# Siyou-Li/u2Tokenizer

Measured on NVIDIA H100. Metric: ct_volumes_per_sec, higher is better.
Workload: dtype bf16

## Files before the change

include/u2b200.h:

```cpp
#ifndef U2B200_H_
#define U2B200_H_

#include <stdint.h>

#if defined(__GNUC__)
#define U2_API __attribute__((visibility("default")))
#else
#define U2_API
#endif

#ifdef __cplusplus
extern "C" {
#endif

#define U2_OK 0
#define U2_ERR_ARG (-1)
#define U2_ERR_CUDA (-2)
#define U2_ERR_UNSUPPORTED (-3)

#define U2_DT_BF16 0
#define U2_DT_F32 1

#define U2_ACT_NONE 0
#define U2_ACT_GELU 1
// ... 97 lines not shown
} u2_rope_desc;
U2_API int u2_rope_bf16(void* x, const u2_rope_desc* desc, void* stream);

U2_API int u2_decode_attention_bf16(const void* q, const void* k_cache, const void* v_cache, void* out,
                                    int32_t B, int32_t Hq, int32_t Hkv, int32_t dh, int32_t Tmax, int32_t T,
                                    const int32_t* T_dev, int64_t ldq, int64_t ldo, float scale, int32_t T_per_seq,
                                    const int32_t* kv_src, int64_t ld_kv_src, void* stream);
U2_API int u2_decode_attention_window_bf16(const void* q, const void* k_cache, const void* v_cache, void* out,
                                           int32_t B, int32_t Hq, int32_t Hkv, int32_t dh, int32_t Tmax, int32_t T,
                                           const int32_t* T_dev, int64_t ldq, int64_t ldo, float scale,
                                           int32_t T_per_seq, const int32_t* kv_src, int64_t ld_kv_src,
                                           int32_t window, void* stream);

typedef struct u2_gemv_desc {
  int32_t B, N, K;
  int64_t ldx, ldw, ldy, ldr;
  int32_t y_dtype;
  const void* residual;
  const float* norm_gamma;
  float norm_eps;
  int32_t silu_pair;
} u2_gemv_desc;
U2_API int u2_gemv_bf16(const void* x, const void* w, void* y, const u2_gemv_desc* desc, void* stream);
U2_API int u2_argmax_f32(const float* logits, int64_t* out, uint64_t* scratch, int32_t B, int32_t V, int64_t ld,
                         void* stream);

#define U2_DLIN_STREAMK128 0
#define U2_DLIN_TILES64 1
typedef struct u2_dlinear_desc {
  int32_t B, N, K;
  int64_t ldx, ldw, ldy, ldr, ldxg;
  int32_t y_dtype;
  float* ws;
  int32_t* counters;
  const float* ssq_in;
  float eps;
  const void* residual;
  int32_t silu_pair;
  const float* gamma_next;
  void* xg;
  float* ssq_out;
  float* ssq_zero;
  int32_t pdl;
  void* dbg;
  int64_t ws_elems;
  const int32_t* dep_flags;
  int32_t dep_shift;
  int32_t* out_flags;
  int32_t sched;
} u2_dlinear_desc;
U2_API int u2_dlinear_bf16(const void* x, const void* w, void* y, const u2_dlinear_desc* desc, void* stream);
U2_API int64_t u2_dlinear_ws_elems(int32_t N, int32_t K);
typedef struct u2_dlinear_next {
  int32_t pre_stages;
  int32_t lookahead_units;
  int32_t n;
  const void* w[2];
  int32_t N[2], K[2];
  int64_t ldw[2];
  int32_t units[2];
} u2_dlinear_next;
U2_API int u2_dlinear_multi_bf16(const void* const* x, const void* const* w, void* const* y,
                                 const u2_dlinear_desc* descs, int32_t n_ops, uint32_t* gridbar,
                                 const int32_t* step_dev, int32_t pdl, const u2_dlinear_next* next, void* stream);
U2_API int u2_decode_embed_bf16(const int64_t* ids, const void* table, const float* gamma, void* x, void* xg,
                                float* ssq, float* ssq_zero, int32_t* step_counter, int32_t B, int32_t E,
                                int64_t vocab, void* stream);

typedef struct u2_fused_decode_desc {
  int32_t B, Hq, Hkv, dh, Tmax, pos;
  const int32_t* pos_dev;
  int64_t ldq, ldo;
  const float* q_norm_w;
  const float* k_norm_w;
  float eps;
  const float* inv_freq;
  float scale;
  int32_t kv_splits;
  int32_t pdl;
  int32_t pos_per_seq;
  const int32_t* kv_src;
  int64_t ld_kv_src;
  int32_t window;
} u2_fused_decode_desc;
U2_API int u2_decode_attention_fused_bf16(const void* qkv, void* k_cache, void* v_cache, void* out,
                                          const u2_fused_decode_desc* desc, void* stream);

U2_API int u2_topk_rows_f32(const float* scores, int64_t* out_idx, int32_t rows, int32_t T, int32_t K, int64_t ld,
                            int64_t idx_offset_per_row, void* stream);

typedef struct u2_fa_desc {
  int32_t B, H, Sq, Sk, dh;
  float scale;
  int64_t q_sb, q_ss, q_sh;
  int64_t k_sb, k_ss, k_sh;
  int64_t v_sb, v_ss, v_sh;
  int64_t out_sb, out_ss;
  float* lse;
} u2_fa_desc;
U2_API int u2_flash_attention_d64_bf16(const void* q, const void* k, const void* v, void* out, const u2_fa_desc* desc,
                                       void* stream);

U2_API int u2_sample_f32(const float* logits, int64_t* out, int32_t B, int32_t V, int64_t ld, float temperature,
                         int32_t top_k, float top_p, uint64_t seed, const int32_t* step_dev, int32_t step,
                         void* stream);

typedef struct u2_sample_params {
  float temperature;
  int32_t top_k;
  float top_p;
  int32_t reserved;
  uint64_t seed;
} u2_sample_params;
U2_API int u2_sample_dev_f32(const float* logits, int64_t* out, int32_t B, int32_t V, int64_t ld,
                             const u2_sample_params* params_dev, const int32_t* step_dev, int32_t step, void* stream);

#define U2_LP_MAX_EOS 8
#define U2_LP_MAX_BAD_WORDS 256
#define U2_LP_MAX_BAD_TOKENS 2048
typedef struct u2_logits_proc_params {
  float penalty;
  float inv_penalty;
  int32_t ngram;
  int32_t min_new;
  int32_t n_eos;
  int32_t n_bad;
  int32_t eos[U2_LP_MAX_EOS];
  int32_t bad_off[U2_LP_MAX_BAD_WORDS + 1];
  int32_t bad_tok[U2_LP_MAX_BAD_TOKENS];
} u2_logits_proc_params;
U2_API int u2_logits_process_f32(float* logits, int32_t B, int32_t V, int64_t ld, const int64_t* ids, int32_t* hist,
                                 int64_t ld_hist, int32_t hist_cap, const u2_logits_proc_params* params_dev,
                                 const int32_t* step_dev, int32_t step, void* stream);

#define U2_BEAM_MAX_BEAMS 16
#define U2_BEAM_MAX_EOS 8
#define U2_BEAM_MAX_KEEP 144
typedef struct u2_beam_params {
  double length_penalty;
  int32_t num_beams;
  int32_t beams_to_keep;
  int32_t early_stopping;
  int32_t max_new_tokens;
  int32_t n_eos;
  int32_t reserved;
  int32_t eos[U2_BEAM_MAX_EOS];
} u2_beam_params;
typedef struct u2_beam_step_desc {
  const u2_beam_params* params;
  int32_t prompts, V;
  const float* cand_val;
  const int32_t* cand_tok;
  float* running;
  float* fin_score;
  int32_t* fin_info;
  int32_t* flags;
  int64_t* ids;
  int32_t* rec;
  int64_t ld_rec;
  int32_t rec_rows;
  int32_t* kv_src;
  int64_t ld_kv_src;
  const int32_t* pos_dev;
  int32_t* hist;
  int64_t ld_hist;
  int32_t hist_cap;
// ... 50 lines not shown
```

u2tokenizer_b200/_lib.py:

```python
from __future__ import annotations

import ctypes as C
from pathlib import Path

_LIB_PATH = Path(__file__).resolve().parent / "libu2b200.so"
_lib = None


class GemmDesc(C.Structure):
    _fields_ = [
        ("M", C.c_int32), ("N", C.c_int32), ("K", C.c_int32),
        ("zi", C.c_int32), ("zo", C.c_int32), ("b_zi_div", C.c_int32),
        ("lda", C.c_int64), ("a_stride_zi", C.c_int64), ("a_stride_zo", C.c_int64),
        ("ldb", C.c_int64), ("b_stride_zi", C.c_int64), ("b_stride_zo", C.c_int64),
        ("ldc", C.c_int64), ("c_stride_zi", C.c_int64), ("c_stride_zo", C.c_int64),
        ("c_dtype", C.c_int32), ("alpha", C.c_float),
        ("bias", C.c_void_p),
        ("act", C.c_int32),
        ("residual", C.c_void_p),
        ("ldr", C.c_int64),
        ("res_row_mod", C.c_int32),
        ("row_div", C.c_int32), ("row_stride", C.c_int32), ("row_off", C.c_int32),
        ("block_n", C.c_int32),
        ("a_mn", C.c_int32), ("b_mn", C.c_int32),
        ("epi_op", C.c_int32),
        ("rowvec", C.c_void_p),
        ("rv_stride_zi", C.c_int64), ("rv_stride_zo", C.c_int64),
        ("mul", C.c_void_p),
    ]


class SoftmaxDesc(C.Structure):
    _fields_ = [
        ("in_s0", C.c_int64), ("in_s1", C.c_int64), ("in_s2", C.c_int64),
        ("out_s0", C.c_int64), ("out_s1", C.c_int64), ("out_s2", C.c_int64),
        ("n0", C.c_int32), ("H", C.c_int32), ("S", C.c_int32), ("n", C.c_int32),
        ("scale", C.c_float),
        ("rel_bias", C.c_void_p),
        ("rel_max", C.c_int32),
        ("causal", C.c_int32), ("causal_off", C.c_int32),
        ("zero_pad_to", C.c_int32),
        ("window", C.c_int32),
    ]


class RopeDesc(C.Structure):
    _fields_ = [
        ("rows", C.c_int64), ("ld", C.c_int64),
        ("dh", C.c_int32), ("n_q_heads", C.c_int32), ("n_k_heads", C.c_int32), ("n_v_heads", C.c_int32),
        ("q_norm_w", C.c_void_p), ("k_norm_w", C.c_void_p),
        ("eps", C.c_float),
        ("inv_freq", C.c_void_p),
        ("pos0", C.c_int32), ("pos_div", C.c_int32), ("pos_mod", C.c_int32),
        ("pos0_dev", C.c_void_p),
        ("k_cache", C.c_void_p), ("v_cache", C.c_void_p),
        ("Tmax", C.c_int32), ("rows_per_batch", C.c_int32),
        ("pos0_per_batch", C.c_int32),
    ]


class GemvDesc(C.Structure):
    _fields_ = [
        ("B", C.c_int32), ("N", C.c_int32), ("K", C.c_int32),
        ("ldx", C.c_int64), ("ldw", C.c_int64), ("ldy", C.c_int64), ("ldr", C.c_int64),
        ("y_dtype", C.c_int32),
        ("residual", C.c_void_p),
        ("norm_gamma", C.c_void_p),
        ("norm_eps", C.c_float),
        ("silu_pair", C.c_int32),
    ]


class DlinearDesc(C.Structure):
    _fields_ = [
        ("B", C.c_int32), ("N", C.c_int32), ("K", C.c_int32),
        ("ldx", C.c_int64), ("ldw", C.c_int64), ("ldy", C.c_int64), ("ldr", C.c_int64), ("ldxg", C.c_int64),
        ("y_dtype", C.c_int32),
        ("ws", C.c_void_p), ("counters", C.c_void_p),
        ("ssq_in", C.c_void_p),
        ("eps", C.c_float),
        ("residual", C.c_void_p),
        ("silu_pair", C.c_int32),
        ("gamma_next", C.c_void_p),
        ("xg", C.c_void_p),
        ("ssq_out", C.c_void_p),
        ("ssq_zero", C.c_void_p),
        ("pdl", C.c_int32),
        ("dbg", C.c_void_p),
        ("ws_elems", C.c_int64),
        ("dep_flags", C.c_void_p), ("dep_shift", C.c_int32), ("out_flags", C.c_void_p),
        ("sched", C.c_int32),
    ]


class FusedDecodeDesc(C.Structure):
    _fields_ = [
        ("B", C.c_int32), ("Hq", C.c_int32), ("Hkv", C.c_int32), ("dh", C.c_int32), ("Tmax", C.c_int32),
        ("pos", C.c_int32),
        ("pos_dev", C.c_void_p),
        ("ldq", C.c_int64), ("ldo", C.c_int64),
        ("q_norm_w", C.c_void_p), ("k_norm_w", C.c_void_p),
        ("eps", C.c_float),
        ("inv_freq", C.c_void_p),
        ("scale", C.c_float),
        ("kv_splits", C.c_int32), ("pdl", C.c_int32),
        ("pos_per_seq", C.c_int32),
        ("kv_src", C.c_void_p), ("ld_kv_src", C.c_int64),
        ("window", C.c_int32),
    ]


class DlinearNext(C.Structure):
    _fields_ = [
        ("pre_stages", C.c_int32), ("lookahead_units", C.c_int32), ("n", C.c_int32),
        ("w", C.c_void_p * 2),
        ("N", C.c_int32 * 2), ("K", C.c_int32 * 2),
        ("ldw", C.c_int64 * 2),
        ("units", C.c_int32 * 2),
    ]


class FaDesc(C.Structure):
    _fields_ = [
        ("B", C.c_int32), ("H", C.c_int32), ("Sq", C.c_int32), ("Sk", C.c_int32), ("dh", C.c_int32),
        ("scale", C.c_float),
        ("q_sb", C.c_int64), ("q_ss", C.c_int64), ("q_sh", C.c_int64),
        ("k_sb", C.c_int64), ("k_ss", C.c_int64), ("k_sh", C.c_int64),
        ("v_sb", C.c_int64), ("v_ss", C.c_int64), ("v_sh", C.c_int64),
        ("out_sb", C.c_int64), ("out_ss", C.c_int64),
        ("lse", C.c_void_p),
    ]


class LogprobDesc(C.Structure):
    _fields_ = [
        ("R", C.c_int32), ("V", C.c_int32), ("E", C.c_int32),
        ("ldh", C.c_int64), ("ldw", C.c_int64),
        ("labels", C.c_void_p), ("ws", C.c_void_p), ("ws_bytes", C.c_int64),
        ("lse", C.c_void_p), ("logit_sum", C.c_void_p), ("nll_acc", C.c_void_p),
    ]


class PreprocessInfo(C.Structure):
    _fields_ = [
        ("a_min", C.c_double), ("a_max", C.c_double),
        ("lo", C.c_int32 * 3), ("hi", C.c_int32 * 3), ("out", C.c_int32 * 3),
        ("sigma", C.c_float * 3), ("tail", C.c_int32 * 3), ("status", C.c_int32),
    ]


class PreprocessDesc(C.Structure):
    _fields_ = [
        ("D", C.c_int32), ("H", C.c_int32), ("W", C.c_int32), ("target", C.c_int32), ("pad_depth", C.c_int32),
        ("lower_pct", C.c_double), ("upper_pct", C.c_double),
        ("ws", C.c_void_p), ("ws_bytes", C.c_int64),
    ]


class SoftmaxBwdDesc(C.Structure):
    _fields_ = [
        ("p_s0", C.c_int64), ("p_s1", C.c_int64), ("p_s2", C.c_int64),
        ("dp_s0", C.c_int64), ("dp_s1", C.c_int64), ("dp_s2", C.c_int64),
        ("ds_s0", C.c_int64), ("ds_s1", C.c_int64), ("ds_s2", C.c_int64),
        ("n0", C.c_int32), ("H", C.c_int32), ("S", C.c_int32), ("n", C.c_int32),
        ("zero_pad_to", C.c_int32),
    ]


class AdamWDesc(C.Structure):
    _fields_ = [
        ("lr", C.c_float), ("beta1", C.c_float), ("beta2", C.c_float), ("eps", C.c_float), ("weight_decay", C.c_float),
        ("step", C.c_int32),
        ("grad_scale", C.c_void_p),
        ("seed", C.c_uint64), ("index_offset", C.c_int64),
    ]


class LoraDesc(C.Structure):
    _fields_ = [
        ("M", C.c_int32), ("K", C.c_int32), ("r", C.c_int32), ("n_adapters", C.c_int32),
        ("ldx", C.c_int64), ("ldu", C.c_int64),
        ("scale", C.c_float), ("p", C.c_float),
        ("seed", C.c_uint64),
        ("stream", C.c_int32 * 3),
        ("accumulate", C.c_int32),
    ]


LP_MAX_EOS, LP_MAX_BAD_WORDS, LP_MAX_BAD_TOKENS = 8, 256, 2048


# ... 154 lines not shown
```

u2tokenizer_b200/csrc/attn_small.cu:

```cuda
#include <cooperative_groups.h>
#include <cuda_bf16.h>
#include <math.h>

#include <type_traits>

#include "host_util.h"
#include "u2b200.h"

namespace u2 {

__device__ __forceinline__ float wsum(float v) {
#pragma unroll
  for (int o = 16; o > 0; o >>= 1) v += __shfl_xor_sync(0xffffffffu, v, o);
  return v;
}
__device__ __forceinline__ float wmax(float v) {
#pragma unroll
  for (int o = 16; o > 0; o >>= 1) v = fmaxf(v, __shfl_xor_sync(0xffffffffu, v, o));
  return v;
}

__global__ void __launch_bounds__(128)
temporal_attention_kernel(const __nv_bfloat16* __restrict__ qkv, __nv_bfloat16* __restrict__ out, int C, int N,
                          int H, int dh, long long ld_qkv, long long ld_out, float scale,
// ... 701 lines not shown
#pragma unroll
      for (int i = 0; i < kEpl; ++i) acc[g][i] *= corr;
      m[g] = mx;
    }
#pragma unroll
    for (int jj = 0; jj < 32; ++jj) {
      float vf[kEpl];
      if (t0 + jj == pos) {
#pragma unroll
        for (int i = 0; i < kEpl; ++i) vf[i] = __bfloat162float(s_vnew[le * kEpl + i]);
      } else if constexpr (kEpl == 4) {
        const float2 x = __bfloat1622float2(*reinterpret_cast<const __nv_bfloat162*>(&vw[jj][0]));
        const float2 y = __bfloat1622float2(*reinterpret_cast<const __nv_bfloat162*>(&vw[jj][1]));
        vf[0] = x.x; vf[1] = x.y; vf[2] = y.x; vf[3] = y.y;
      } else if constexpr (kEpl == 2) {
        const float2 x = __bfloat1622float2(*reinterpret_cast<const __nv_bfloat162*>(&vw[jj][0]));
        vf[0] = x.x; vf[1] = x.y;
      } else {
        vf[0] = __uint_as_float(vw[jj][0] << 16);
      }
#pragma unroll
      for (int g = 0; g < kG; ++g) {
        const float pj = __shfl_sync(0xffffffffu, p[g], jj);
#pragma unroll
        for (int i = 0; i < kEpl; ++i) acc[g][i] += pj * vf[i];
      }
    }
    t0 += S * kW * 32;
    if (t0 < T) request(t0);
  }
#pragma unroll
  for (int g = 0; g < kG; ++g) {
    if (lane == 0) {
      s_m[warp][g] = m[g];
      s_l[warp][g] = l[g];
    }
    if (kLanes == 32 || lane < kLanes) {
#pragma unroll
      for (int i = 0; i < kEpl; ++i) s_acc[warp][g][lane * kEpl + i] = acc[g][i];
    }
  }
  __syncthreads();
  for (int idx = threadIdx.x; idx < kG * kDh; idx += blockDim.x) {
    const int g = idx / kDh, e = idx - g * kDh;
    float gm = -INFINITY;
#pragma unroll
    for (int w = 0; w < kW; ++w) gm = fmaxf(gm, s_m[w][g]);
    float gl = 0.f, o = 0.f;
#pragma unroll
    for (int w = 0; w < kW; ++w) {
      if (s_m[w][g] != -INFINITY) {
        const float f = __expf(s_m[w][g] - gm);
        gl += s_l[w][g] * f;
        o += s_acc[w][g][e] * f;
      }
    }
    c_o[g][e] = o;
    if (e == 0) {
      c_m[g] = gm;
      c_l[g] = gl;
    }
  }
  cluster.sync();
  if (rank == 0) {
    for (int idx = threadIdx.x; idx < kG * kDh; idx += blockDim.x) {
      const int g = idx / kDh, e = idx - g * kDh;
      float gm = -INFINITY;
      for (int r = 0; r < S; ++r) gm = fmaxf(gm, *cluster.map_shared_rank(&c_m[g], r));
      float gl = 0.f, o = 0.f;
      for (int r = 0; r < S; ++r) {
        const float mr = *cluster.map_shared_rank(&c_m[g], r);
        if (mr != -INFINITY) {
          const float f = __expf(mr - gm);
          gl += *cluster.map_shared_rank(&c_l[g], r) * f;
          o += *cluster.map_shared_rank(&c_o[g][e], r) * f;
        }
      }
      a.out[(long long)b * a.ldo + (long long)(hk * kG + g) * kDh + e] = __float2bfloat16(o / gl);
    }
  }
  cluster.sync();
}

template <int kDh, int kG, bool kInd, bool kWin>
static int launch_fused_decode_split(const FusedArgsT<kInd, kWin>& a, dim3 grid, bool pdl, cudaStream_t st) {
  cudaLaunchConfig_t cfg = {};
  cfg.gridDim = grid;
  cfg.blockDim = dim3(256);
  cfg.dynamicSmemBytes = 0;
  cfg.stream = st;
  cudaLaunchAttribute attr[2];
  attr[0].id = cudaLaunchAttributeClusterDimension;
  attr[0].val.clusterDim.x = 1;
  attr[0].val.clusterDim.y = 1;
  attr[0].val.clusterDim.z = grid.z;
  attr[1].id = cudaLaunchAttributeProgrammaticStreamSerialization;
  attr[1].val.programmaticStreamSerializationAllowed = 1;
  cfg.attrs = attr;
  cfg.numAttrs = pdl ? 2 : 1;
  cudaError_t e = cudaLaunchKernelEx(&cfg, fused_decode_attention_split_kernel<kDh, kG, kInd, kWin>, a);
  if (e != cudaSuccess) return set_error(U2_ERR_CUDA, "decode_attention_fused (split-KV) launch: %s", cudaGetErrorString(e));
  return U2_OK;
}

template <int kDh, bool kInd, bool kWin = false>
static int launch_fused_decode(const FusedArgsT<kInd, kWin>& a, int G, dim3 grid, bool pdl, cudaStream_t st) {
  if (grid.z > 1) {
    switch (G) {
      case 1: return launch_fused_decode_split<kDh, 1, kInd, kWin>(a, grid, pdl, st);
      case 2: return launch_fused_decode_split<kDh, 2, kInd, kWin>(a, grid, pdl, st);
      case 4: return launch_fused_decode_split<kDh, 4, kInd, kWin>(a, grid, pdl, st);
      case 8: return launch_fused_decode_split<kDh, 8, kInd, kWin>(a, grid, pdl, st);
      default: return set_error(U2_ERR_UNSUPPORTED, "decode_attention_fused: Hq/Hkv = %d (supported 1, 2, 4, 8)", G);
    }
  }
  switch (G) {
    case 1: fused_decode_attention_kernel<kDh, 1, kInd, kWin><<<grid, FaCfg<kDh, 1>::kWarps * 32, 0, st>>>(a); break;
    case 2: fused_decode_attention_kernel<kDh, 2, kInd, kWin><<<grid, FaCfg<kDh, 2>::kWarps * 32, 0, st>>>(a); break;
    case 4: fused_decode_attention_kernel<kDh, 4, kInd, kWin><<<grid, FaCfg<kDh, 4>::kWarps * 32, 0, st>>>(a); break;
    case 8: fused_decode_attention_kernel<kDh, 8, kInd, kWin><<<grid, FaCfg<kDh, 8>::kWarps * 32, 0, st>>>(a); break;
    default: return set_error(U2_ERR_UNSUPPORTED, "decode_attention_fused: Hq/Hkv = %d (supported 1, 2, 4, 8)", G);
  }
  return U2_OK;
}

template <int kDh>
static int launch_fused_decode(const FusedDecodeWinArgs& a, int G, dim3 grid, bool pdl, cudaStream_t st) {
  if (a.window > 0) {
    if (a.kv_src) return launch_fused_decode<kDh, true, true>(a, G, grid, pdl, st);
    return launch_fused_decode<kDh, false, true>(a, G, grid, pdl, st);
  }
  if (a.kv_src) return launch_fused_decode<kDh, true>(static_cast<const FusedDecodeIndArgs&>(a), G, grid, pdl, st);
  return launch_fused_decode<kDh, false>(static_cast<const FusedDecodeArgs&>(a), G, grid, pdl, st);
}

}

extern "C" U2_API int u2_decode_attention_fused_bf16(const void* qkv, void* k_cache, void* v_cache, void* out,
                                                     const u2_fused_decode_desc* d, void* stream) {
  using namespace u2;
  if (!qkv || !k_cache || !v_cache || !out || !d || !d->inv_freq) return set_error(U2_ERR_ARG, "decode_attention_fused: null pointer");
  if (d->Hkv <= 0 || d->Hq % d->Hkv || d->Hq / d->Hkv > kFaMaxG)
    return set_error(U2_ERR_UNSUPPORTED, "decode_attention_fused: Hq/Hkv must be an integer <= %d", kFaMaxG);
  if (!d->pos_dev && (d->pos < 0 || d->pos >= d->Tmax)) return set_error(U2_ERR_ARG, "decode_attention_fused: position outside the cache");
  if (d->pos_per_seq && !d->pos_dev) return set_error(U2_ERR_ARG, "decode_attention_fused: pos_per_seq needs pos_dev");
  if (d->window < 0) return set_error(U2_ERR_ARG, "decode_attention_fused: window %d < 0", d->window);
  FusedDecodeWinArgs a;
  a.qkv = CBF(qkv); a.ldq = d->ldq;
  a.kc = BF(k_cache); a.vc = BF(v_cache);
  a.out = BF(out); a.ldo = d->ldo;
  a.Hq = d->Hq; a.Hkv = d->Hkv; a.Tmax = d->Tmax;
  a.pos_dev = d->pos_dev; a.pos_per_seq = d->pos_per_seq != 0; a.pos_host = d->pos;
  a.q_norm_w = d->q_norm_w; a.k_norm_w = d->k_norm_w; a.eps = d->eps;
  a.inv_freq = d->inv_freq; a.scale = d->scale;
  a.kv_src = d->kv_src; a.ld_src = d->ld_kv_src;
  a.window = d->window;
  if (a.kv_src && a.ld_src < d->Tmax) return set_error(U2_ERR_ARG, "decode_attention_fused: kv_src row stride < Tmax");
  const int splits = d->kv_splits > 1 ? d->kv_splits : 1;
  if (splits != 1 && splits != 2 && splits != 4 && splits != 8)
    return set_error(U2_ERR_ARG, "decode_attention_fused: kv_splits must be 0/1, 2, 4 or 8 (portable cluster sizes)");
  dim3 grid((unsigned)d->Hkv, (unsigned)d->B, (unsigned)splits);
  const int G = d->Hq / d->Hkv;
  int rc;
  switch (d->dh) {
    case 32: rc = launch_fused_decode<32>(a, G, grid, d->pdl != 0, ST(stream)); break;
    case 64: rc = launch_fused_decode<64>(a, G, grid, d->pdl != 0, ST(stream)); break;
    case 96: rc = launch_fused_decode<96>(a, G, grid, d->pdl != 0, ST(stream)); break;
    case 128: rc = launch_fused_decode<128>(a, G, grid, d->pdl != 0, ST(stream)); break;
    default: return set_error(U2_ERR_UNSUPPORTED, "decode_attention_fused: head_dim %d (supported 32/64/96/128)", d->dh);
  }
  if (rc) return rc;
  U2_CHECK_LAUNCH("decode_attention_fused");
  return U2_OK;
}
```

u2tokenizer_b200/engine.py:

```python
from __future__ import annotations

import math
from dataclasses import asdict, dataclass, replace
from typing import Dict, List, Optional, Tuple

import torch

from . import _lib, ops
from .geometry import Geometry

BF16, F32 = torch.bfloat16, torch.float32
REL_MAX = 512


def _pad8(n: int) -> int:
    return (n + 7) // 8 * 8


@dataclass(frozen=True)
class LogitsProcessors:
    repetition_penalty: float = 1.0
    no_repeat_ngram_size: int = 0
    min_new_tokens: int = 0
    eos_token_ids: Tuple[int, ...] = ()
# ... 540 lines not shown

    def token_logps(self, hidden: torch.Tensor, labels: torch.Tensor, *, want_lse=False, want_logit_sum=False,
                    nll_acc: Optional[torch.Tensor] = None):
        shp = labels.shape
        h2 = hidden.reshape(-1, hidden.shape[-1])
        if not h2.is_contiguous():
            h2 = h2.contiguous()
        logp, lse, lsum = ops.lmhead_logprob(h2, self.lm_head, labels.reshape(-1).contiguous(), want_lse=want_lse,
                                             want_logit_sum=want_logit_sum, nll_acc=nll_acc)
        rs = lambda t: None if t is None else t.view(shp)
        return rs(logp), rs(lse), rs(lsum)

    def _decode_buffers(self, B: int):
        g = self.g
        key = ("dec", B)
        if getattr(self, "_dec_key", None) != key:
            if getattr(self, "_gen_state", None) is not None:
                self._gen_state["graph"] = None
            hq, hkv, dh, I, E = g.num_attention_heads, g.num_key_value_heads, g.head_dim, g.intermediate_size, g.hidden_size
            d = self.dev
            self._dec = dict(
                x=torch.empty(B, E, device=d, dtype=BF16), qkv=torch.empty(B, (hq + 2 * hkv) * dh, device=d, dtype=BF16),
                ctx=torch.empty(B, hq * dh, device=d, dtype=BF16), act=torch.empty(B, I, device=d, dtype=BF16),
                logits=torch.empty(B, g.vocab_size, device=d, dtype=F32), ids=torch.zeros(B, 1, device=d, dtype=torch.int64),
                xg=torch.empty(B, E, device=d, dtype=BF16), xg2=torch.empty(B, E, device=d, dtype=BF16),
                ssq_a=torch.zeros(16, device=d, dtype=F32),
                ssq_b=torch.zeros(16, device=d, dtype=F32))
            max_n = max(g.vocab_size, 2 * I, (hq + 2 * hkv) * dh, E)
            shapes = [((hq + 2 * hkv) * dh, E), (E, hq * dh), (2 * I, E), (E, I), (g.vocab_size, E)]
            wse = max(ops.dlinear_ws_elems(n, k) for n, k in shapes)
            self._dec["ws"] = ops.dlinear_new_ws(wse, device=d, lead=(2,))
            self._dec["counters"] = torch.zeros(2, (max_n + 63) // 64 + 8, device=d, dtype=torch.int32)
            self._dec["flags"] = torch.zeros(g.num_hidden_layers, 4, 256, device=d, dtype=torch.int32)
            self._dec["gridbar"] = torch.zeros(4 * g.num_hidden_layers, device=d, dtype=torch.int32)
            self._dec["step"] = torch.zeros(1, device=d, dtype=torch.int32)
            self._dec_key = key
        return self._dec

    def reset_decode_state(self, B: int):
        bufs = self._decode_buffers(B)
        for k in ("gridbar", "step", "counters", "ssq_a", "ssq_b", "flags"):
            bufs[k].zero_()
        bufs["ws"].view(torch.int32).fill_(-1)

    def _kv_splits(self, B: int) -> int:
        import os
        env = os.environ.get("U2_ATTN_SPLIT", "auto")
        if env != "auto":
            return max(1, int(env))
        pairs = B * self.g.num_key_value_heads
        s = 8
        while s > 1 and pairs * s > max(self.num_sms, pairs):
            s //= 2
        return s

    def _use_tc_decode(self, B: int) -> bool:
        g = self.g
        dims = (g.hidden_size, g.intermediate_size, g.num_attention_heads * g.head_dim)
        return self.decode_impl == "tcgen05" and B <= 16 and all(k % 64 == 0 for k in dims)

    def _decode_rows(self) -> int:
        tc_rows = 16
        return tc_rows if self._use_tc_decode(tc_rows) else 8

    def decode_step_tc(self, cache: "KVCache", req: Optional[GenerateRequest] = None) -> torch.Tensor:
        g = self.g
        B = cache.batch
        hq, hkv, dh = g.num_attention_heads, g.num_key_value_heads, g.head_dim
        bufs = self._decode_buffers(B)
        x, qkv, ctx, act, logits, ids, xg_a, xg_b = (bufs[k] for k in ("x", "qkv", "ctx", "act", "logits", "ids", "xg", "xg2"))
        ssq_a, ssq_b, ws, cnt, flags = bufs["ssq_a"], bufs["ssq_b"], bufs["ws"], bufs["counters"], bufs["flags"]
        gridbar, step = bufs["gridbar"], bufs["step"]
        eps = g.rms_norm_eps
        nl = len(self.layers)
        c0 = dict(ws=ws[0], counters=cnt[0], sched=self.dl_sched)
        c1 = dict(ws=ws[1], counters=cnt[1], sched=self.dl_sched)
        ops.decode_embed(ids, self.embed, self.layers[0]["ln1"], x, xg_b, ssq_b, ssq_a, step)
        ops.dlinear(xg_b, self.layers[0]["wqkv"], qkv, ssq_in=ssq_b, eps=eps, pdl=self.pdl, **c1)
        for li, w in enumerate(self.layers):
            ops.decode_attention_fused(qkv, cache.k[li], cache.v[li], ctx, B=B, Hq=hq, Hkv=hkv, dh=dh, Tmax=cache.max_len,
                                       inv_freq=self.inv_freq, scale=1.0 / math.sqrt(dh), pos_dev=cache.length_dev,
                                       q_norm_w=w["qn"], k_norm_w=w["kn"], eps=eps, kv_splits=self._kv_splits(B),
                                       pdl=self.pdl and self.attn_pdl, pos_per_seq=True, kv_src=cache.kv_src,
                                       window=g.window)
            last = li + 1 == nl
            g_next = self.final_norm if last else self.layers[li + 1]["ln1"]
            fl = flags[li] if (self.multi_op and self.fine_deps) else [None] * 4
            dep = lambda i, shift: dict(dep_flags=fl[i], dep_shift=shift) if fl[i] is not None else {}
            chain = [
                (ctx, w["wo"], x, dict(residual=x, gamma_next=w["ln2"], xg=xg_a, ssq_out=ssq_a, ssq_zero=ssq_b,
                                       out_flags=fl[0], **c0)),
                (xg_a, w["wgu"], act, dict(ssq_in=ssq_a, eps=eps, silu_pair=True, out_flags=fl[1], **dep(0, 1), **c1)),
                (act, w["wdown"], x, dict(residual=x, gamma_next=g_next, xg=xg_b, ssq_out=ssq_b, ssq_zero=ssq_a,
                                          out_flags=fl[2], **dep(1, 0), **c0)),
                (xg_b, self.lm_head, logits, dict(ssq_in=ssq_b, eps=eps, **dep(2, 1), **c1)) if last else
                (xg_b, self.layers[li + 1]["wqkv"], qkv, dict(ssq_in=ssq_b, eps=eps, **dep(2, 1), **c1)),
            ]
            if self.multi_op:
                nxt = () if (last or self.l2_next_units < 0) else (
                    (self.layers[li + 1]["wo"], 1 << 20), (self.layers[li + 1]["wgu"], self.l2_next_units))
                ops.dlinear_multi(chain, gridbar=gridbar[li * 4:(li + 1) * 4], step_dev=step, pdl=self.pdl,
                                  lookahead_units=self.l2_lookahead_units, next_weights=nxt,
                                  pre_stages=self.pre_stages)
            else:
                for (xi, wi, yi, kw) in chain:
                    ops.dlinear(xi, wi, yi, pdl=self.pdl, **kw)
        self._pick_next(logits, ids.view(B), bufs["step"], req)
        cache.advance_device()
        return logits

    def _pick_next(self, logits: torch.Tensor, ids_out: torch.Tensor, step_dev: Optional[torch.Tensor],
                   req: Optional[GenerateRequest], step: int = 0):
        if req is not None and req.beam is not None:
            return self._beam_pick(logits, ids_out, step_dev, req, step)
        if req is not None and req.processors is not None:
            blk = self._param_block("logits processors", ops.logits_proc_params, self.g.vocab_size,
                                    **asdict(req.processors))
            ops.logits_process(logits, blk, ids_out, self._gen_state["hist"], step=step, step_dev=step_dev)
        if req is None or req.sampling is None:
            ops.argmax(logits, ids_out)
        else:
            ops.sample_dev(logits, self._param_block("sampling parameters", ops.sample_params, *req.sampling), ids_out,
                           step=step, step_dev=step_dev)

    def _param_block(self, what: str, make, *args, **kw) -> torch.Tensor:
        host = (args, kw)
        blk = self._param_blocks.get(what)
        if blk is None:
            self._param_blocks[what] = blk = [host, make(self.dev, *args, **kw)]
        elif blk[0] != host:
            if torch.cuda.is_current_stream_capturing():
                raise RuntimeError(f"{what} changed inside a CUDA-graph capture")
            make(self.dev, *args, out=blk[1], **kw)
            blk[0] = host
        return blk[1]

    def _beam_pick(self, logits: torch.Tensor, ids_out: torch.Tensor, step_dev: Optional[torch.Tensor],
                   req: GenerateRequest, step: int):
        st = self._gen_state
        bs, bm = st["beam"], req.beam
        blk = self._param_block("beam search parameters", ops.beam_params, num_beams=bm.num_beams,
                                length_penalty=bm.length_penalty, early_stopping=bm.early_stopping,
                                max_new_tokens=req.max_new_tokens, eos_token_ids=req.eos_token_id)
        lp = ops.log_softmax(logits, bs["lp"])
        if req.processors is not None:
            pblk = self._param_block("logits processors", ops.logits_proc_params, self.g.vocab_size,
                                     **asdict(req.processors))
            ops.logits_process(lp, pblk, ids_out, st["hist"], step=step, step_dev=step_dev)
        ops.beam_topk(lp, bs["running"], bs["flags"], blk, bs["cand_val"], bs["cand_tok"])
        ops.beam_step(blk, bs, ids_out, st["cache"].kv_src, st["cache"].length_dev, V=logits.shape[1],
                      hist=st.get("hist"), step=step, step_dev=step_dev)

    def decode_step(self, cache: "KVCache", req: Optional[GenerateRequest] = None) -> torch.Tensor:
        g = self.g
        B = cache.batch
        if self._use_tc_decode(B):
            return self.decode_step_tc(cache, req)
        hq, hkv, dh = g.num_attention_heads, g.num_key_value_heads, g.head_dim
        bufs = self._decode_buffers(B)
        x, qkv, ctx, act, logits, ids = (bufs[k] for k in ("x", "qkv", "ctx", "act", "logits", "ids"))
        ops.embed_splice(ids, self.embed, None, out=x)
        nqkv = (hq + 2 * hkv) * dh
        for li, w in enumerate(self.layers):
            ops.gemv(x, w["wqkv"], qkv, norm_gamma=w["ln1"], norm_eps=g.rms_norm_eps)
            ops.rope(qkv, rows=B, ld=nqkv, dh=dh, n_q=hq, n_k=hkv, n_v=hkv, inv_freq=self.inv_freq, q_norm_w=w["qn"],
                     k_norm_w=w["kn"], eps=g.rms_norm_eps, pos0=0, pos_div=1, pos_mod=1, pos0_dev=cache.length_dev,
                     k_cache=cache.k[li], v_cache=cache.v[li], Tmax=cache.max_len, rows_per_batch=1, pos0_per_batch=True)
# ... 244 lines not shown
```

u2tokenizer_b200/ops.py:

```python
from __future__ import annotations

import ctypes as C
from typing import Optional

import torch

from . import _lib
from ._lib import GemmDesc

BF16 = torch.bfloat16
F32 = torch.float32

ACT_NONE, ACT_GELU, ACT_SILU = 0, 1, 2
DT_BF16, DT_F32 = 0, 1


def _stream() -> int:
    return torch.cuda.current_stream().cuda_stream


def _ptr(t: Optional[torch.Tensor]) -> Optional[int]:
    return None if t is None else t.data_ptr()


# ... 345 lines not shown
                                         _stream()), "u2_argmax_f32")
    return out


def _dlinear_desc(x, w, out, *, ws, counters, ssq_in=None, eps=1e-6, residual=None, silu_pair=False, gamma_next=None,
                  xg=None, ssq_out=None, ssq_zero=None, pdl=True, dbg=None, sched=0, dep_flags=None, dep_shift=1,
                  out_flags=None):
    _need_cuda(x, w, out, ws, counters, ssq_in, residual, gamma_next, xg, ssq_out, ssq_zero)
    d = _lib.DlinearDesc()
    d.B, d.N, d.K = x.shape[0], w.shape[0], w.shape[1]
    if counters.numel() < (d.N + 63) // 64 + (ssq_out is not None):
        raise ValueError("dlinear counters too small: ceil(N / 64) int32, + 1 with ssq_out")
    d.ws_elems = ws.numel()
    d.ldx, d.ldw, d.ldy = x.stride(0), w.stride(0), out.stride(0)
    d.ldr = residual.stride(0) if residual is not None else 0
    d.ldxg = xg.stride(0) if xg is not None else 0
    d.y_dtype = DT_BF16 if out.dtype == BF16 else DT_F32
    d.ws, d.counters = ws.data_ptr(), counters.data_ptr()
    d.ssq_in = _ptr(ssq_in)
    d.eps = eps
    d.residual = _ptr(residual)
    d.silu_pair = int(silu_pair)
    d.gamma_next = _ptr(gamma_next)
    d.xg = _ptr(xg)
    d.ssq_out = _ptr(ssq_out)
    d.ssq_zero = _ptr(ssq_zero)
    d.pdl = int(pdl)
    d.dbg = _ptr(dbg)
    _need_cuda(dep_flags, out_flags)
    d.dep_flags, d.dep_shift, d.out_flags = _ptr(dep_flags), dep_shift, _ptr(out_flags)
    d.sched = int(sched)
    return d


def dlinear_ws_elems(N: int, K: int) -> int:
    return int(_lib.load().u2_dlinear_ws_elems(N, K))


def dlinear_new_ws(n_elems: int, device="cuda", lead=()) -> torch.Tensor:
    return torch.full((*lead, max(int(n_elems), 4)), -1, device=device, dtype=torch.int32).view(F32)


def dlinear(x: torch.Tensor, w: torch.Tensor, out: torch.Tensor, **kw):
    d = _dlinear_desc(x, w, out, **kw)
    _lib.check(_lib.load().u2_dlinear_bf16(x.data_ptr(), w.data_ptr(), out.data_ptr(), C.byref(d), _stream()),
               "u2_dlinear_bf16")
    return out


def dlinear_multi(ops_list, *, gridbar: torch.Tensor, step_dev: torch.Tensor, pdl: bool = True,
                  lookahead_units: int = 0, next_weights=(), pre_stages: int = 0):
    n = len(ops_list)
    descs = (_lib.DlinearDesc * n)()
    xs, ws_, ys = (C.c_void_p * n)(), (C.c_void_p * n)(), (C.c_void_p * n)()
    for i, (x, w, out, kw) in enumerate(ops_list):
        descs[i] = _dlinear_desc(x, w, out, **kw)
        xs[i], ws_[i], ys[i] = x.data_ptr(), w.data_ptr(), out.data_ptr()
    _need_cuda(gridbar, step_dev)
    nx = _lib.DlinearNext()
    nx.lookahead_units = lookahead_units
    nx.pre_stages = pre_stages
    nx.n = len(next_weights)
    for j, (wn, units) in enumerate(next_weights):
        _need_cuda(wn)
        nx.w[j], nx.N[j], nx.K[j], nx.ldw[j], nx.units[j] = wn.data_ptr(), wn.shape[0], wn.shape[1], wn.stride(0), units
    _lib.check(_lib.load().u2_dlinear_multi_bf16(xs, ws_, ys, descs, n, gridbar.data_ptr(), step_dev.data_ptr(),
                                                 int(pdl), C.byref(nx), _stream()), "u2_dlinear_multi_bf16")


def decode_embed(ids: torch.Tensor, table: torch.Tensor, gamma: torch.Tensor, x: torch.Tensor, xg: torch.Tensor,
                 ssq: torch.Tensor, ssq_zero: Optional[torch.Tensor], step_counter: Optional[torch.Tensor] = None):
    _need_cuda(ids, table, gamma, x, xg, ssq, ssq_zero, step_counter)
    _lib.check(_lib.load().u2_decode_embed_bf16(ids.data_ptr(), table.data_ptr(), gamma.data_ptr(), x.data_ptr(),
                                                xg.data_ptr(), ssq.data_ptr(), _ptr(ssq_zero), _ptr(step_counter),
                                                ids.numel(),
                                                table.shape[1], table.shape[0], _stream()), "u2_decode_embed_bf16")
    return x


def decode_attention_fused(qkv: torch.Tensor, k_cache: torch.Tensor, v_cache: torch.Tensor, out: torch.Tensor, *,
                           B: int, Hq: int, Hkv: int, dh: int, Tmax: int, inv_freq: torch.Tensor, scale: float,
                           pos: int = 0, pos_dev=None, q_norm_w=None, k_norm_w=None, eps: float = 1e-6, kv_splits: int = 1,
                           pdl: bool = False, pos_per_seq: bool = False, kv_src: Optional[torch.Tensor] = None,
                           window: int = 0):
    _need_cuda(qkv, k_cache, v_cache, out, inv_freq, pos_dev, q_norm_w, k_norm_w, kv_src)
    _check_kv_src(kv_src, B, Tmax)
    d = _lib.FusedDecodeDesc()
    d.B, d.Hq, d.Hkv, d.dh, d.Tmax, d.pos = B, Hq, Hkv, dh, Tmax, pos
    d.pos_dev = _ptr(pos_dev)
    d.ldq, d.ldo = qkv.stride(0), out.stride(0)
    d.q_norm_w, d.k_norm_w, d.eps = _ptr(q_norm_w), _ptr(k_norm_w), eps
    d.inv_freq = inv_freq.data_ptr()
    d.scale = scale
    d.kv_splits = int(kv_splits)
    d.pdl = 1 if pdl else 0
    d.pos_per_seq = 1 if pos_per_seq else 0
    d.kv_src = _ptr(kv_src)
    d.ld_kv_src = kv_src.stride(0) if kv_src is not None else 0
    d.window = int(window or 0)
    _lib.check(_lib.load().u2_decode_attention_fused_bf16(qkv.data_ptr(), k_cache.data_ptr(), v_cache.data_ptr(),
                                                          out.data_ptr(), C.byref(d), _stream()),
               "u2_decode_attention_fused_bf16")
    return out


def topk_rows(scores: torch.Tensor, k: int, idx_offset_per_row: int = 0) -> torch.Tensor:
    _need_cuda(scores)
    if scores.dtype != F32 or scores.stride(1) != 1:
        raise TypeError("topk_rows expects fp32 rows")
    rows, T = scores.shape
    out = torch.empty(rows, k, device=scores.device, dtype=torch.int64)
    _lib.check(_lib.load().u2_topk_rows_f32(scores.data_ptr(), out.data_ptr(), rows, T, k, scores.stride(0),
                                            idx_offset_per_row, _stream()), "u2_topk_rows_f32")
    return out


def flash_attention_d64(q: torch.Tensor, k: torch.Tensor, v: torch.Tensor, out: torch.Tensor, scale: float,
                        lse: Optional[torch.Tensor] = None):
    _need_cuda(q, k, v, out)
    B, Sq, H, dh = q.shape
    Sk = k.shape[1]
    if dh != 64 or q.stride(3) != 1 or k.stride(3) != 1 or v.stride(3) != 1 or out.stride(2) != 1 or v.shape != k.shape:
        raise ValueError("flash_attention_d64: head_dim must be 64 with a contiguous last dim, v shaped like k")
    d = _lib.FaDesc()
    d.B, d.H, d.Sq, d.Sk, d.dh, d.scale = B, H, Sq, Sk, dh, scale
    d.q_sb, d.q_ss, d.q_sh = q.stride(0), q.stride(1), q.stride(2)
    d.k_sb, d.k_ss, d.k_sh = k.stride(0), k.stride(1), k.stride(2)
    d.v_sb, d.v_ss, d.v_sh = v.stride(0), v.stride(1), v.stride(2)
    d.out_sb, d.out_ss = out.stride(0), out.stride(1)
    _need_cuda(lse)
    if lse is not None and (lse.dtype != F32 or not lse.is_contiguous() or lse.numel() != B * H * Sq):
        raise ValueError("flash_attention_d64: lse must be contiguous fp32 [B, H, Sq]")
    d.lse = _ptr(lse)
    _lib.check(_lib.load().u2_flash_attention_d64_bf16(q.data_ptr(), k.data_ptr(), v.data_ptr(), out.data_ptr(),
                                                       C.byref(d), _stream()), "u2_flash_attention_d64_bf16")
    return out


def sample(logits: torch.Tensor, out: Optional[torch.Tensor] = None, *, temperature: float = 1.0, top_k: int = 50,
           top_p: float = 1.0, seed: int = 0, step: int = 0, step_dev=None) -> torch.Tensor:
    _need_cuda(logits, step_dev)
    B, V = logits.shape
    if out is None:
        out = torch.empty(B, device=logits.device, dtype=torch.int64)
    _lib.check(_lib.load().u2_sample_f32(logits.data_ptr(), out.data_ptr(), B, V, logits.stride(0), temperature,
                                         int(top_k), float(top_p), int(seed) & ((1 << 64) - 1), _ptr(step_dev),
                                         int(step), _stream()), "u2_sample_f32")
    return out


def sample_params(device, temperature: float, top_k: int, top_p: float, seed: int,
                  out: Optional[torch.Tensor] = None) -> torch.Tensor:
    import struct
    if not temperature > 0:
        raise ValueError("sample: temperature must be > 0")
    if not 0 < top_p <= 1:
        raise ValueError("sample: top_p must be in (0, 1]")
    raw = struct.pack("<fifiQ", float(temperature), int(top_k), float(top_p), 0, int(seed) & ((1 << 64) - 1))
    host = torch.frombuffer(bytearray(raw), dtype=torch.uint8)
    if out is None:
        return host.to(device)
    out.copy_(host)
    return out


def sample_dev(logits: torch.Tensor, params: torch.Tensor, out: Optional[torch.Tensor] = None, *, step: int = 0,
               step_dev=None) -> torch.Tensor:
    _need_cuda(logits, params, step_dev)
    B, V = logits.shape
    if params.dtype != torch.uint8 or params.numel() != 24:
        raise ValueError("sample_dev: params must be the 24-byte block of sample_params()")
    if out is None:
        out = torch.empty(B, device=logits.device, dtype=torch.int64)
    _lib.check(_lib.load().u2_sample_dev_f32(logits.data_ptr(), out.data_ptr(), B, V, logits.stride(0), params.data_ptr(),
                                             _ptr(step_dev), int(step), _stream()), "u2_sample_dev_f32")
    return out


def logits_proc_params(device, vocab_size: int, *, repetition_penalty: float = 1.0, no_repeat_ngram_size: int = 0,
                       min_new_tokens: int = 0, eos_token_ids=(), bad_words_ids=(),
                       out: Optional[torch.Tensor] = None) -> torch.Tensor:
    import numpy as np
# ... 190 lines not shown
```

Before: 2.166.

## Add packed 128-thread split-KV decode attention kernel with KV prefetch

Adds a new split-KV decode attention kernel that runs 128 threads per block with a minimum of 4 blocks per SM. Each warp handles two of eight virtual warp slots, and the kernel issues L2 prefetches of the KV rows before the PDL wait plus L1 prefetches inside the main loop. It is selected for head dims 96 and 128 with group sizes 1, 2 and 4, and the engine now enables it by default. The aim is higher occupancy and latency hiding for memory-bound decode. The costs are more register pressure under the launch bounds, larger per-block shared memory for the eight-slot accumulators, and a maximum-shared carveout that shrinks L1.

```diff
diff --git a/include/u2b200.h b/include/u2b200.h
--- a/include/u2b200.h
+++ b/include/u2b200.h
@@ -203,6 +203,7 @@
   const int32_t* kv_src;
   int64_t ld_kv_src;
   int32_t window;
+  int32_t packed;
 } u2_fused_decode_desc;
 U2_API int u2_decode_attention_fused_bf16(const void* qkv, void* k_cache, void* v_cache, void* out,
                                           const u2_fused_decode_desc* desc, void* stream);
diff --git a/u2tokenizer_b200/_lib.py b/u2tokenizer_b200/_lib.py
--- a/u2tokenizer_b200/_lib.py
+++ b/u2tokenizer_b200/_lib.py
@@ -106,7 +106,7 @@
         ("kv_splits", C.c_int32), ("pdl", C.c_int32),
         ("pos_per_seq", C.c_int32),
         ("kv_src", C.c_void_p), ("ld_kv_src", C.c_int64),
-        ("window", C.c_int32),
+        ("window", C.c_int32), ("packed", C.c_int32),
     ]
 
 
diff --git a/u2tokenizer_b200/csrc/attn_small.cu b/u2tokenizer_b200/csrc/attn_small.cu
--- a/u2tokenizer_b200/csrc/attn_small.cu
+++ b/u2tokenizer_b200/csrc/attn_small.cu
@@ -807,6 +807,276 @@
   cluster.sync();
 }
 
+constexpr int kPkThreads = 128;
+constexpr int kPkMinBlocks = 4;
+
+__device__ __forceinline__ void prefetch_l2(const void* p) {
+  asm volatile("prefetch.global.L2 [%0];" ::"l"(p));
+}
+__device__ __forceinline__ void prefetch_l1(const void* p) {
+  asm volatile("prefetch.global.L1 [%0];" ::"l"(p));
+}
+
+template <int kDh, int kG, bool kInd, bool kWin = false>
+__global__ void __launch_bounds__(kPkThreads, kPkMinBlocks)
+fused_decode_attention_packed_kernel(const FusedArgsT<kInd, kWin> a) {
+  namespace cg = cooperative_groups;
+  cg::cluster_group cluster = cg::this_cluster();
+  constexpr int kW = 8;
+  constexpr int kWarps = kPkThreads / 32;
+  constexpr int kEpl = PvMap<kDh>::kEpl;
+  constexpr int kLanes = PvMap<kDh>::kLanes;
+  constexpr int kVw = (kEpl + 1) / 2;
+  constexpr int kKc = kDh / 8;
+  constexpr int kVc = 16;
+  static_assert((kDh / 8) % kKc == 0 && 32 % kVc == 0, "chunking");
+  const int S = (int)gridDim.z, rank = (int)blockIdx.z;
+  const int hk = blockIdx.x, b = blockIdx.y;
+  const int warp = threadIdx.x >> 5, lane = threadIdx.x & 31;
+  const int le = kLanes == 32 ? lane : min(lane, kLanes - 1);
+  asm volatile("griddepcontrol.launch_dependents;" ::: "memory");
+  const int pos = a.pos_dev ? a.pos_dev[a.pos_per_seq ? b : 0] : a.pos_host;
+  const int T = min(pos + 1, a.Tmax);
+  const int lo = window_lo<kWin>(a, pos);
+  __shared__ __align__(16) float s_q[kG][kDh];
+  __shared__ __align__(16) __nv_bfloat16 s_knew[kDh];
+  __shared__ __align__(16) __nv_bfloat16 s_vnew[kDh];
+  __shared__ float s_m[kW][kG], s_l[kW][kG];
+  __shared__ float s_acc[kW][kG][kDh];
+  __shared__ float c_m[kG], c_l[kG];
+  __shared__ __align__(16) float c_o[kG][kDh];
+
+  const __nv_bfloat16* row = a.qkv + (long long)b * a.ldq;
+  __nv_bfloat16* kbase = a.kc + ((long long)b * a.Hkv + hk) * a.Tmax * kDh;
+  __nv_bfloat16* vbase = a.vc + ((long long)b * a.Hkv + hk) * a.Tmax * kDh;
+  const long long row_elems = (long long)a.Hkv * a.Tmax * kDh;
+  const int first = (lo & ~31) + rank * 32, stride = S * kW * 32;
+
+  for (int w = warp; w < kW; w += kWarps) {
+    for (int t0 = first + w * S * 32; t0 < T; t0 += stride) {
+      const int t = min(t0 + lane, T - 1);
+      const long long off = (long long)t * kDh + kv_src_delta<kInd>(a, b, t, pos, row_elems);
+#pragma unroll
+      for (int o = 0; o < kDh; o += 64) {
+        prefetch_l2(kbase + off + o);
+        prefetch_l2(vbase + off + o);
+      }
+      prefetch_l2(kbase + off + kDh - 1);
+      prefetch_l2(vbase + off + kDh - 1);
+    }
+  }
+  asm volatile("griddepcontrol.wait;" ::: "memory");
+
+  for (int job = warp; job < kG + 2; job += kWarps) {
+    if (job == kG) {
+      norm_rope_head<kDh>(row + (long long)(a.Hq + hk) * kDh, a.k_norm_w, a.eps, a.inv_freq, pos, 1.f, nullptr, s_knew, lane);
+      __syncwarp();
+      if (rank == 0)
+        for (int e = lane; e < kDh; e += 32) kbase[(long long)pos * kDh + e] = s_knew[e];
+    } else if (job == kG + 1) {
+      const __nv_bfloat16* v = row + (long long)(a.Hq + a.Hkv + hk) * kDh;
+      for (int e = lane; e < kDh; e += 32) {
+        const __nv_bfloat16 x = v[e];
+        s_vnew[e] = x;
+        if (rank == 0) vbase[(long long)pos * kDh + e] = x;
+      }
+    } else {
+      norm_rope_head<kDh>(row + (long long)(hk * kG + job) * kDh, a.q_norm_w, a.eps, a.inv_freq, pos, a.scale, s_q[job],
+                          nullptr, lane);
+    }
+  }
+  __syncthreads();
+
+  for (int w = warp; w < kW; w += kWarps) {
+    float m[kG], l[kG], acc[kG][kEpl];
+#pragma unroll
+    for (int g = 0; g < kG; ++g) {
+      m[g] = -INFINITY;
+      l[g] = 0.f;
+#pragma unroll
+      for (int i = 0; i < kEpl; ++i) acc[g][i] = 0.f;
+    }
+    for (int t0 = first + w * S * 32; t0 < T; t0 += stride) {
+      const int t = t0 + lane;
+      const int tc = min(t, T - 1);
+      const long long dsrc = kv_src_delta<kInd>(a, b, tc, pos, row_elems);
+      const uint4* kr = reinterpret_cast<const uint4*>(kbase + (long long)tc * kDh + dsrc);
+#pragma unroll
+      for (int o = 0; o < kDh; o += 64) {
+        prefetch_l1(kbase + (long long)tc * kDh + dsrc + o);
+        prefetch_l1(vbase + (long long)tc * kDh + dsrc + o);
+      }
+      prefetch_l1(vbase + (long long)tc * kDh + dsrc + kDh - 1);
+      float s[kG];
+#pragma unroll
+      for (int g = 0; g < kG; ++g) s[g] = 0.f;
+#pragma unroll
+      for (int c0 = 0; c0 < kDh / 8; c0 += kKc) {
+        uint4 u[kKc];
+#pragma unroll
+        for (int c = 0; c < kKc; ++c) u[c] = kr[c0 + c];
+        if (t == pos) {
+#pragma unroll
+          for (int c = 0; c < kKc; ++c) u[c] = reinterpret_cast<const uint4*>(s_knew)[c0 + c];
+        }
+#pragma unroll
+        for (int c = 0; c < kKc; ++c) {
+          const __nv_bfloat162* h2 = reinterpret_cast<const __nv_bfloat162*>(&u[c]);
+          float kf[8];
+#pragma unroll
+          for (int j = 0; j < 4; ++j) {
+            const float2 f2 = __bfloat1622float2(h2[j]);
+            kf[2 * j] = f2.x;
+            kf[2 * j + 1] = f2.y;
+          }
+#pragma unroll
+          for (int g = 0; g < kG; ++g) {
+            const float4 q0 = *reinterpret_cast<const float4*>(&s_q[g][(c0 + c) * 8]);
+            const float4 q1 = *reinterpret_cast<const float4*>(&s_q[g][(c0 + c) * 8 + 4]);
+            s[g] += kf[0] * q0.x + kf[1] * q0.y + kf[2] * q0.z + kf[3] * q0.w + kf[4] * q1.x + kf[5] * q1.y +
+                    kf[6] * q1.z + kf[7] * q1.w;
+          }
+        }
+      }
+      float p[kG];
+      const bool vis = t < T && (!kWin || t >= lo);
+#pragma unroll
+      for (int g = 0; g < kG; ++g) {
+        if (!vis) s[g] = -INFINITY;
+        const float mx = fmaxf(m[g], wmax(s[g]));
+        const float corr = __expf(m[g] - mx);
+        p[g] = vis ? __expf(s[g] - mx) : 0.f;
+        l[g] = l[g] * corr + wsum(p[g]);
+#pragma unroll
+        for (int i = 0; i < kEpl; ++i) acc[g][i] *= corr;
+        m[g] = mx;
+      }
+#pragma unroll 1
+      for (int j0 = 0; j0 < 32; j0 += kVc) {
+        uint32_t vw[kVc][kVw];
+#pragma unroll
+        for (int jj = 0; jj < kVc; ++jj) {
+          const int tj = min(t0 + j0 + jj, T - 1);
+          long long dj = 0;
+          if constexpr (kInd) dj = __shfl_sync(0xffffffffu, dsrc, tj - t0);
+          const __nv_bfloat16* vp = vbase + (long long)tj * kDh + dj + le * kEpl;
+          if constexpr (kEpl == 4) {
+            const uint2 u = *reinterpret_cast<const uint2*>(vp);
+            vw[jj][0] = u.x;
+            vw[jj][1] = u.y;
+          } else if constexpr (kEpl == 2) {
+            vw[jj][0] = *reinterpret_cast<const uint32_t*>(vp);
+          } else {
+            vw[jj][0] = *reinterpret_cast<const unsigned short*>(vp);
+          }
+        }
+#pragma unroll
+        for (int jj = 0; jj < kVc; ++jj) {
+          float vf[kEpl];
+          if (t0 + j0 + jj == pos) {
+#pragma unroll
+            for (int i = 0; i < kEpl; ++i) vf[i] = __bfloat162float(s_vnew[le * kEpl + i]);
+          } else if constexpr (kEpl == 4) {
+            const float2 x = __bfloat1622float2(*reinterpret_cast<const __nv_bfloat162*>(&vw[jj][0]));
+            const float2 y = __bfloat1622float2(*reinterpret_cast<const __nv_bfloat162*>(&vw[jj][1]));
+            vf[0] = x.x; vf[1] = x.y; vf[2] = y.x; vf[3] = y.y;
+          } else if constexpr (kEpl == 2) {
+            const float2 x = __bfloat1622float2(*reinterpret_cast<const __nv_bfloat162*>(&vw[jj][0]));
+            vf[0] = x.x; vf[1] = x.y;
+          } else {
+            vf[0] = __uint_as_float(vw[jj][0] << 16);
+          }
+#pragma unroll
+          for (int g = 0; g < kG; ++g) {
+            const float pj = __shfl_sync(0xffffffffu, p[g], j0 + jj);
+#pragma unroll
+            for (int i = 0; i < kEpl; ++i) acc[g][i] += pj * vf[i];
+          }
+        }
+      }
+    }
+#pragma unroll
+    for (int g = 0; g < kG; ++g) {
+      if (lane == 0) {
+        s_m[w][g] = m[g];
+        s_l[w][g] = l[g];
+      }
+      if (kLanes == 32 || lane < kLanes) {
+#pragma unroll
+        for (int i = 0; i < kEpl; ++i) s_acc[w][g][lane * kEpl + i] = acc[g][i];
+      }
+    }
+  }
+  __syncthreads();
+  for (int idx = threadIdx.x; idx < kG * kDh; idx += blockDim.x) {
+    const int g = idx / kDh, e = idx - g * kDh;
+    float gm = -INFINITY;
+#pragma unroll
+    for (int w = 0; w < kW; ++w) gm = fmaxf(gm, s_m[w][g]);
+    float gl = 0.f, o = 0.f;
+#pragma unroll
+    for (int w = 0; w < kW; ++w) {
+      if (s_m[w][g] != -INFINITY) {
+        const float f = __expf(s_m[w][g] - gm);
+        gl += s_l[w][g] * f;
+        o += s_acc[w][g][e] * f;
+      }
+    }
+    c_o[g][e] = o;
+    if (e == 0) {
+      c_m[g] = gm;
+      c_l[g] = gl;
+    }
+  }
+  cluster.sync();
+  if (rank == 0) {
+    for (int idx = threadIdx.x; idx < kG * kDh; idx += blockDim.x) {
+      const int g = idx / kDh, e = idx - g * kDh;
+      float gm = -INFINITY;
+      for (int r = 0; r < S; ++r) gm = fmaxf(gm, *cluster.map_shared_rank(&c_m[g], r));
+      float gl = 0.f, o = 0.f;
+      for (int r = 0; r < S; ++r) {
+        const float mr = *cluster.map_shared_rank(&c_m[g], r);
+        if (mr != -INFINITY) {
+          const float f = __expf(mr - gm);
+          gl += *cluster.map_shared_rank(&c_l[g], r) * f;
+          o += *cluster.map_shared_rank(&c_o[g][e], r) * f;
+        }
+      }
+      a.out[(long long)b * a.ldo + (long long)(hk * kG + g) * kDh + e] = __float2bfloat16(o / gl);
+    }
+  }
+  cluster.sync();
+}
+
+template <int kDh, int kG, bool kInd, bool kWin>
+static int launch_fused_decode_packed(const FusedArgsT<kInd, kWin>& a, dim3 grid, bool pdl, cudaStream_t st) {
+  auto kern = fused_decode_attention_packed_kernel<kDh, kG, kInd, kWin>;
+  static bool configured = false;
+  if (!configured) {
+    cudaError_t e = cudaFuncSetAttribute(kern, cudaFuncAttributePreferredSharedMemoryCarveout, cudaSharedmemCarveoutMaxShared);
+    if (e != cudaSuccess) return set_error(U2_ERR_CUDA, "decode_attention_fused (packed) carveout: %s", cudaGetErrorString(e));
+    configured = true;
+  }
+  cudaLaunchConfig_t cfg = {};
+  cfg.gridDim = grid;
+  cfg.blockDim = dim3(kPkThreads);
+  cfg.dynamicSmemBytes = 0;
+  cfg.stream = st;
+  cudaLaunchAttribute attr[2];
+  attr[0].id = cudaLaunchAttributeClusterDimension;
+  attr[0].val.clusterDim.x = 1;
+  attr[0].val.clusterDim.y = 1;
+  attr[0].val.clusterDim.z = grid.z;
+  attr[1].id = cudaLaunchAttributeProgrammaticStreamSerialization;
+  attr[1].val.programmaticStreamSerializationAllowed = 1;
+  cfg.attrs = attr;
+  cfg.numAttrs = pdl ? 2 : 1;
+  cudaError_t e = cudaLaunchKernelEx(&cfg, kern, a);
+  if (e != cudaSuccess) return set_error(U2_ERR_CUDA, "decode_attention_fused (packed) launch: %s", cudaGetErrorString(e));
+  return U2_OK;
+}
+
 template <int kDh, int kG, bool kInd, bool kWin>
 static int launch_fused_decode_split(const FusedArgsT<kInd, kWin>& a, dim3 grid, bool pdl, cudaStream_t st) {
   cudaLaunchConfig_t cfg = {};
@@ -829,7 +1099,17 @@
 }
 
 template <int kDh, bool kInd, bool kWin = false>
-static int launch_fused_decode(const FusedArgsT<kInd, kWin>& a, int G, dim3 grid, bool pdl, cudaStream_t st) {
+static int launch_fused_decode(const FusedArgsT<kInd, kWin>& a, int G, dim3 grid, bool pdl, bool packed, cudaStream_t st) {
+  if constexpr (kDh == 96 || kDh == 128) {
+    if (packed && grid.z > 1) {
+      switch (G) {
+        case 1: return launch_fused_decode_packed<kDh, 1, kInd, kWin>(a, grid, pdl, st);
+        case 2: return launch_fused_decode_packed<kDh, 2, kInd, kWin>(a, grid, pdl, st);
+        case 4: return launch_fused_decode_packed<kDh, 4, kInd, kWin>(a, grid, pdl, st);
+        default: break;
+      }
+    }
+  }
   if (grid.z > 1) {
     switch (G) {
       case 1: return launch_fused_decode_split<kDh, 1, kInd, kWin>(a, grid, pdl, st);
@@ -850,13 +1130,13 @@
 }
 
 template <int kDh>
-static int launch_fused_decode(const FusedDecodeWinArgs& a, int G, dim3 grid, bool pdl, cudaStream_t st) {
+static int launch_fused_decode(const FusedDecodeWinArgs& a, int G, dim3 grid, bool pdl, bool packed, cudaStream_t st) {
   if (a.window > 0) {
-    if (a.kv_src) return launch_fused_decode<kDh, true, true>(a, G, grid, pdl, st);
-    return launch_fused_decode<kDh, false, true>(a, G, grid, pdl, st);
-  }
-  if (a.kv_src) return launch_fused_decode<kDh, true>(static_cast<const FusedDecodeIndArgs&>(a), G, grid, pdl, st);
-  return launch_fused_decode<kDh, false>(static_cast<const FusedDecodeArgs&>(a), G, grid, pdl, st);
+    if (a.kv_src) return launch_fused_decode<kDh, true, true>(a, G, grid, pdl, packed, st);
+    return launch_fused_decode<kDh, false, true>(a, G, grid, pdl, packed, st);
+  }
+  if (a.kv_src) return launch_fused_decode<kDh, true>(static_cast<const FusedDecodeIndArgs&>(a), G, grid, pdl, packed, st);
+  return launch_fused_decode<kDh, false>(static_cast<const FusedDecodeArgs&>(a), G, grid, pdl, packed, st);
 }
 
 }
@@ -888,10 +1168,10 @@
   const int G = d->Hq / d->Hkv;
   int rc;
   switch (d->dh) {
-    case 32: rc = launch_fused_decode<32>(a, G, grid, d->pdl != 0, ST(stream)); break;
-    case 64: rc = launch_fused_decode<64>(a, G, grid, d->pdl != 0, ST(stream)); break;
-    case 96: rc = launch_fused_decode<96>(a, G, grid, d->pdl != 0, ST(stream)); break;
-    case 128: rc = launch_fused_decode<128>(a, G, grid, d->pdl != 0, ST(stream)); break;
+    case 32: rc = launch_fused_decode<32>(a, G, grid, d->pdl != 0, d->packed != 0, ST(stream)); break;
+    case 64: rc = launch_fused_decode<64>(a, G, grid, d->pdl != 0, d->packed != 0, ST(stream)); break;
+    case 96: rc = launch_fused_decode<96>(a, G, grid, d->pdl != 0, d->packed != 0, ST(stream)); break;
+    case 128: rc = launch_fused_decode<128>(a, G, grid, d->pdl != 0, d->packed != 0, ST(stream)); break;
     default: return set_error(U2_ERR_UNSUPPORTED, "decode_attention_fused: head_dim %d (supported 32/64/96/128)", d->dh);
   }
   if (rc) return rc;
diff --git a/u2tokenizer_b200/engine.py b/u2tokenizer_b200/engine.py
--- a/u2tokenizer_b200/engine.py
+++ b/u2tokenizer_b200/engine.py
@@ -646,7 +646,7 @@
                                        inv_freq=self.inv_freq, scale=1.0 / math.sqrt(dh), pos_dev=cache.length_dev,
                                        q_norm_w=w["qn"], k_norm_w=w["kn"], eps=eps, kv_splits=self._kv_splits(B),
                                        pdl=self.pdl and self.attn_pdl, pos_per_seq=True, kv_src=cache.kv_src,
-                                       window=g.window)
+                                       window=g.window, packed=True)
             last = li + 1 == nl
             g_next = self.final_norm if last else self.layers[li + 1]["ln1"]
             fl = flags[li] if (self.multi_op and self.fine_deps) else [None] * 4
diff --git a/u2tokenizer_b200/ops.py b/u2tokenizer_b200/ops.py
--- a/u2tokenizer_b200/ops.py
+++ b/u2tokenizer_b200/ops.py
@@ -451,7 +451,7 @@
                            B: int, Hq: int, Hkv: int, dh: int, Tmax: int, inv_freq: torch.Tensor, scale: float,
                            pos: int = 0, pos_dev=None, q_norm_w=None, k_norm_w=None, eps: float = 1e-6, kv_splits: int = 1,
                            pdl: bool = False, pos_per_seq: bool = False, kv_src: Optional[torch.Tensor] = None,
-                           window: int = 0):
+                           window: int = 0, packed: bool = False):
     _need_cuda(qkv, k_cache, v_cache, out, inv_freq, pos_dev, q_norm_w, k_norm_w, kv_src)
     _check_kv_src(kv_src, B, Tmax)
     d = _lib.FusedDecodeDesc()
@@ -467,6 +467,7 @@
     d.kv_src = _ptr(kv_src)
     d.ld_kv_src = kv_src.stride(0) if kv_src is not None else 0
     d.window = int(window or 0)
+    d.packed = 1 if packed else 0
     _lib.check(_lib.load().u2_decode_attention_fused_bf16(qkv.data_ptr(), k_cache.data_ptr(), v_cache.data_ptr(),
                                                           out.data_ptr(), C.byref(d), _stream()),
                "u2_decode_attention_fused_bf16")
```

New measurement: 2.224 (median of 6 runs). 1.03x the previous value.
